# nitishsaDire/objectDetection_ssd

Hardware: NVIDIA B200
Metric: images/sec, SSD300 match + multibox loss fwd+bwd (higher is better)
Workload: dtype f32

## Files before the change

objectdetection_ssd_b200/csrc/common.cuh:

```cuda
#pragma once
#include <cuda_runtime.h>
#include <stdint.h>
#include <stdlib.h>
#include "../../include/ssdhead.h"

#if defined(__CUDA_ARCH__) && (__CUDA_ARCH__ < 1000)
#error "libssdhead is written for sm_100a (B200) only"
#endif

namespace ssdhead {

extern unsigned long long g_launch_count;
inline void count_launch(int n = 1) { g_launch_count += (unsigned long long)n; }

#define SSD_CHECK_CUDA(expr) do { cudaError_t _e = (expr); if (_e != cudaSuccess) return (int)_e; } while (0)
#define SSD_LAUNCH_CHECK() do { cudaError_t _e = cudaGetLastError(); if (_e != cudaSuccess) return (int)_e; } while (0)

static inline bool aligned16(const void* p) { return (reinterpret_cast<uintptr_t>(p) & 15u) == 0; }
static inline size_t round_up(size_t x, size_t a) { return (x + a - 1) / a * a; }

constexpr unsigned FULL = 0xffffffffu;

__device__ __forceinline__ float box_area(const float4 b) {
    return __fmul_rn(__fsub_rn(b.z, b.x), __fsub_rn(b.w, b.y));
// ... 8 lines not shown
    const float uni = __fsub_rn(__fadd_rn(area_a, area_b), inter);
    return __fdiv_rn(inter, uni);
}

__device__ __forceinline__ float iou_sparse(const float4 a, const float area_a, const float4 b, const float area_b) {
    const float lx = fmaxf(a.x, b.x), ly = fmaxf(a.y, b.y);
    const float hx = fminf(a.z, b.z), hy = fminf(a.w, b.w);
    const float dx = fmaxf(__fsub_rn(hx, lx), 0.0f);
    const float dy = fmaxf(__fsub_rn(hy, ly), 0.0f);
    const float inter = __fmul_rn(dx, dy);
    if (inter == 0.0f && area_a >= 0.0f) return 0.0f;
    return __fdiv_rn(inter, __fsub_rn(__fadd_rn(area_a, area_b), inter));
}

__device__ __forceinline__ float4 cxcywh_to_xyxy(const float4 b) {
    const float hw = __fdiv_rn(b.z, 2.0f), hh = __fdiv_rn(b.w, 2.0f);
    return make_float4(__fsub_rn(b.x, hw), __fsub_rn(b.y, hh), __fadd_rn(b.x, hw), __fadd_rn(b.y, hh));
}
__device__ __forceinline__ float4 xyxy_to_cxcywh(const float4 b) {
    return make_float4(__fdiv_rn(__fadd_rn(b.z, b.x), 2.0f), __fdiv_rn(__fadd_rn(b.w, b.y), 2.0f),
                       __fsub_rn(b.z, b.x), __fsub_rn(b.w, b.y));
}
__device__ __forceinline__ float4 encode_box(const float4 c, const float4 p) {
    return make_float4(__fdiv_rn(__fsub_rn(c.x, p.x), __fdiv_rn(p.z, 10.0f)),
                       __fdiv_rn(__fsub_rn(c.y, p.y), __fdiv_rn(p.w, 10.0f)),
                       __fmul_rn(logf(__fdiv_rn(c.z, p.z)), 5.0f),
                       __fmul_rn(logf(__fdiv_rn(c.w, p.w)), 5.0f));
}
__device__ __forceinline__ float4 decode_box(const float4 g, const float4 p) {
    return make_float4(__fadd_rn(__fdiv_rn(__fmul_rn(g.x, p.z), 10.0f), p.x),
                       __fadd_rn(__fdiv_rn(__fmul_rn(g.y, p.w), 10.0f), p.y),
                       __fmul_rn(expf(__fdiv_rn(g.z, 5.0f)), p.z),
                       __fmul_rn(expf(__fdiv_rn(g.w, 5.0f)), p.w));
}

__device__ __forceinline__ float fast_exp_ftz(float d) {
    float r;
    asm("ex2.approx.ftz.f32 %0, %1;" : "=f"(r) : "f"(__fmul_rn(d, 1.4426950408889634f)));
    return r;
}

__device__ __forceinline__ uint32_t float_order_key(float f) {
    f = __fadd_rn(f, 0.0f);
    const uint32_t u = __float_as_uint(f);
    return (u & 0x80000000u) ? ~u : (u | 0x80000000u);
}

__device__ __forceinline__ uint32_t smem_u32(const void* p) { return (uint32_t)__cvta_generic_to_shared(p); }

__device__ __forceinline__ void mbar_init(uint64_t* bar, uint32_t count) {
    asm volatile("mbarrier.init.shared::cta.b64 [%0], %1;" :: "r"(smem_u32(bar)), "r"(count) : "memory");
}
__device__ __forceinline__ void mbar_fence_init() {
    asm volatile("fence.mbarrier_init.release.cluster;" ::: "memory");
}
__device__ __forceinline__ void mbar_expect_tx(uint64_t* bar, uint32_t bytes) {
    asm volatile("mbarrier.arrive.expect_tx.shared::cta.b64 _, [%0], %1;" :: "r"(smem_u32(bar)), "r"(bytes) : "memory");
}
__device__ __forceinline__ void mbar_arrive(uint64_t* bar) {
    asm volatile("mbarrier.arrive.shared::cta.b64 _, [%0];" :: "r"(smem_u32(bar)) : "memory");
}
__device__ __forceinline__ void mbar_wait(uint64_t* bar, uint32_t parity) {
    asm volatile(
        "{\n\t.reg .pred p;\n\t"
        "WAIT_%=:\n\t"
        "mbarrier.try_wait.parity.shared::cta.b64 p, [%0], %1;\n\t"
        "@p bra DONE_%=;\n\t"
        "bra WAIT_%=;\n\t"
        "DONE_%=:\n\t}"
        :: "r"(smem_u32(bar)), "r"(parity) : "memory");
}
__device__ __forceinline__ void bulk_g2s(void* smem_dst, const void* gmem_src, uint32_t bytes, uint64_t* bar) {
    asm volatile("cp.async.bulk.shared::cluster.global.mbarrier::complete_tx::bytes [%0], [%1], %2, [%3];"
                 :: "r"(smem_u32(smem_dst)), "l"(gmem_src), "r"(bytes), "r"(smem_u32(bar)) : "memory");
}
__device__ __forceinline__ void bulk_s2g(void* gmem_dst, const void* smem_src, uint32_t bytes) {
    asm volatile("cp.async.bulk.global.shared::cta.bulk_group [%0], [%1], %2;"
                 :: "l"(gmem_dst), "r"(smem_u32(smem_src)), "r"(bytes) : "memory");
}
__device__ __forceinline__ void bulk_commit() { asm volatile("cp.async.bulk.commit_group;" ::: "memory"); }
__device__ __forceinline__ void bulk_wait_read_all() { asm volatile("cp.async.bulk.wait_group.read 0;" ::: "memory"); }
__device__ __forceinline__ void bulk_wait_all() { asm volatile("cp.async.bulk.wait_group 0;" ::: "memory"); }
__device__ __forceinline__ void fence_proxy_async_smem() { asm volatile("fence.proxy.async.shared::cta;" ::: "memory"); }

__device__ __forceinline__ uint64_t ld_cg_u64(const unsigned long long* p) {
    unsigned long long v;
    asm volatile("ld.global.cg.u64 %0, [%1];" : "=l"(v) : "l"(p) : "memory");
    return v;
}
__device__ __forceinline__ uint64_t ld_relaxed_gpu_u64(const unsigned long long* p) {
    unsigned long long v;
    asm volatile("ld.relaxed.gpu.global.u64 %0, [%1];" : "=l"(v) : "l"(p) : "memory");
    return v;
}
__device__ __forceinline__ int ld_relaxed_gpu_s32(const int* p) {
    int v;
    asm volatile("ld.relaxed.gpu.global.s32 %0, [%1];" : "=r"(v) : "l"(p) : "memory");
    return v;
}
__device__ __forceinline__ unsigned int ld_acquire_gpu_u32(const unsigned int* p) {
    unsigned int v;
    asm volatile("ld.acquire.gpu.global.u32 %0, [%1];" : "=r"(v) : "l"(p) : "memory");
    return v;
}
__device__ __forceinline__ void st_relaxed_gpu_u64(unsigned long long* p, unsigned long long v) {
    asm volatile("st.relaxed.gpu.global.u64 [%0], %1;" :: "l"(p), "l"(v) : "memory");
}
__device__ __forceinline__ unsigned short ld_cg_u16(const unsigned short* p) {
    unsigned short v;
    asm volatile("ld.global.cg.u16 %0, [%1];" : "=h"(v) : "l"(p) : "memory");
    return v;
}
__device__ __forceinline__ uint4 ld_cg_v4(const uint4* p) {
    uint4 v;
    asm volatile("ld.global.cg.v4.u32 {%0, %1, %2, %3}, [%4];" : "=r"(v.x), "=r"(v.y), "=r"(v.z), "=r"(v.w) : "l"(p) : "memory");
    return v;
}
__device__ __forceinline__ int ld_cg_s32(const int* p) {
    int v;
    asm volatile("ld.global.cg.s32 %0, [%1];" : "=r"(v) : "l"(p) : "memory");
    return v;
}

__device__ __forceinline__ void pdl_wait() { asm volatile("griddepcontrol.wait;" ::: "memory"); }
__device__ __forceinline__ void pdl_trigger() { asm volatile("griddepcontrol.launch_dependents;" ::: "memory"); }

template <bool COOP = false, typename... KArgs, typename... Args>
static inline cudaError_t launch_pdl(void (*kernel)(KArgs...), dim3 grid, dim3 block, size_t smem, cudaStream_t st, Args... args)
{
    cudaLaunchConfig_t cfg = {};
    cfg.gridDim = grid;
    cfg.blockDim = block;
    cfg.dynamicSmemBytes = smem;
    cfg.stream = st;
    cudaLaunchAttribute attr[2];
    attr[0].id = cudaLaunchAttributeProgrammaticStreamSerialization;
    attr[0].val.programmaticStreamSerializationAllowed = 1;
    attr[1].id = cudaLaunchAttributeCooperative;
    attr[1].val.cooperative = 1;
    cfg.attrs = attr;
    cfg.numAttrs = COOP ? 2 : 1;
    return cudaLaunchKernelEx(&cfg, kernel, KArgs(args)...);
}

struct MatchWs {
    unsigned long long* best_key;
    unsigned int* tile_counter;
    int* npos_acc;
    unsigned int* image_counter;
    unsigned long long* arrive_total;
};
static inline MatchWs match_ws(void* ws, int B, int sumG)
{
    uintptr_t w = (uintptr_t)ws;
    MatchWs m;
    m.best_key = (unsigned long long*)w;          w += round_up((size_t)sumG * 8, 16);
    m.tile_counter = (unsigned int*)w;            w += round_up((size_t)B * 4, 16);
    m.npos_acc = (int*)w;                         w += round_up((size_t)B * 4, 16);
    m.image_counter = (unsigned int*)w;
    m.arrive_total = (unsigned long long*)(w + 8);
    return m;
}
static inline size_t match_ws_bytes(int B, int sumG) { return (uintptr_t)match_ws(nullptr, B, sumG).image_counter + 16; }

__device__ __forceinline__ void st_release_sys_u64(unsigned long long* p, unsigned long long v) {
    asm volatile("st.release.sys.global.u64 [%0], %1;" :: "l"(p), "l"(v) : "memory");
// ... 32 lines not shown
```

objectdetection_ssd_b200/csrc/loss.cu:

```cuda
#include <algorithm>
#include <tuple>
#include <type_traits>
#include "common.cuh"

namespace ssdhead {

#ifdef SSDHEAD_PHASE_TIMES
__device__ long long g_phase_loss[16];
#define LPHASE(i) do { if (blockIdx.x == 0 && threadIdx.x == 0) g_phase_loss[i] = clock64(); } while (0)
__device__ long long g_cta[1024][12];
__device__ unsigned long long g_gt[8];
__device__ __forceinline__ unsigned long long gtimer() { unsigned long long v; asm volatile("mov.u64 %0, %globaltimer;" : "=l"(v)); return v; }
#define GMARK_MAX(i) do { if (threadIdx.x == 0) atomicMax(&g_gt[i], gtimer()); } while (0)
#define GMARK_MIN(i) do { if (threadIdx.x == 0) atomicMin(&g_gt[i], gtimer()); } while (0)
#else
#define LPHASE(i) do { } while (0)
#define GMARK_MAX(i) do { } while (0)
#define GMARK_MIN(i) do { } while (0)
#endif

template <int C, bool FAST = false>
__device__ __forceinline__ float row_cross_entropy(const float* __restrict__ row, int c)
{
    float x[C];
#pragma unroll
    for (int q = 0; q < C; ++q) x[q] = row[q];
    float m = x[0];
#pragma unroll
    for (int q = 1; q < C; ++q) m = fmaxf(m, x[q]);
    float s = 0.0f, xc = 0.0f;
#pragma unroll
    for (int q = 0; q < C; ++q) {
        const float d = __fsub_rn(x[q], m);
        s = __fadd_rn(s, FAST ? fast_exp_ftz(d) : expf(d));
        if (q == c) xc = d;
    }
    const float ce = __fsub_rn(logf(s), xc);
    return __fadd_rn(ce, 0.0f);
}

struct FusedMatch {
    const float4* gt_xyxy;
    const float* gt_cls;
    const int* gt_off;
    const float4* pri_xyxy;
    int P, bg_class;
    float pos_iou;
    uint8_t* cls_u8;
    unsigned long long* best_key;
    int* npos_acc;
    unsigned short* obj_u16;
    const float* seed_lb;
    int sumG;
};

struct FusedPre {
    float4 pb;
    float4 gbox;
    float gcls;
    int b, p;
    int b_first, b_last, off0, G;
};

__device__ __forceinline__ FusedPre fused_prefetch_bp(const FusedMatch& m, int b, int p, bool valid)
{
    FusedPre r;
    const int lane = threadIdx.x & 31;
    r.b = valid ? b : -1;
    r.p = valid ? p : 0;
    r.b_first = (int)__reduce_min_sync(FULL, valid ? (unsigned)r.b : 0x7fffffffu);
    r.b_last = __reduce_max_sync(FULL, r.b);
    r.pb = m.pri_xyxy[r.p];
    r.off0 = 0; r.G = 0;
    r.gbox = make_float4(0.f, 0.f, 0.f, 0.f);
    r.gcls = 0.0f;
    if (r.b_last >= 0) {
        r.off0 = m.gt_off[r.b_first];
        r.G = m.gt_off[r.b_first + 1] - r.off0;
        if (lane < min(r.G, 32)) { r.gbox = m.gt_xyxy[r.off0 + lane]; r.gcls = m.gt_cls[r.off0 + lane]; }
    }
    return r;
}

__device__ __forceinline__ FusedPre fused_prefetch(const FusedMatch& m, unsigned row, bool valid)
{
    const int b = (int)(row / (unsigned)m.P);
    return fused_prefetch_bp(m, b, (int)(row - (unsigned)b * (unsigned)m.P), valid);
}

template <bool MULTI = false>
__device__ __forceinline__ void fused_match_rows(const FusedMatch& m, unsigned row, bool valid, const FusedPre& pre)
{
    const int lane = threadIdx.x & 31;
    if (pre.b_last < 0) return;
    const int b = pre.b, p = pre.p;
    const float4 pb = pre.pb;
    const float pa = box_area(pb);
    if (MULTI && pre.b_last - pre.b_first >= 2) {
        if (valid) {
            const int off0 = m.gt_off[b], G = m.gt_off[b + 1] - off0;
            float bst = 0.0f;
            int obj_b = 0;
            float cls_b = G > 0 ? m.gt_cls[off0] : (float)m.bg_class;
            for (int g = 0; g < G; ++g) {
                const float4 gb = m.gt_xyxy[off0 + g];
                const float dx = __fsub_rn(fminf(gb.z, pb.z), fmaxf(gb.x, pb.x));
                const float dy = __fsub_rn(fminf(gb.w, pb.w), fmaxf(gb.y, pb.y));
                float v = 0.0f;
                if (dx > 0.0f && dy > 0.0f) {
                    const float inter = __fmul_rn(dx, dy);
                    v = __fdiv_rn(inter, __fsub_rn(__fadd_rn(box_area(gb), pa), inter));
                    if (v > bst) { bst = v; cls_b = m.gt_cls[off0 + g]; obj_b = g; }
                }
                if (v != 0.0f || p == 0)
                    atomicMax(&m.best_key[off0 + g],
                              ((unsigned long long)(__float_as_uint(v) | 0x80000000u) << 32) | (unsigned long long)(0xffffffffu - (uint32_t)p));
            }
            const bool hit = (G > 0) && !(bst < m.pos_iou);
            const int c = hit ? (int)cls_b : m.bg_class;
            m.cls_u8[row] = (uint8_t)c;
            if (m.obj_u16) m.obj_u16[row] = (unsigned short)obj_b;
            if (c != m.bg_class) atomicAdd(&m.npos_acc[b], 1);
        }
        return;
    }
    float best = 0.0f;
    int g_mine = 0, obj_mine = 0;
    float cls_mine = (float)m.bg_class;
    float wx1 = pb.x, wy1 = pb.y, wx2 = pb.z, wy2 = pb.w;
#pragma unroll
    for (int d = 16; d > 0; d >>= 1) {
        wx1 = fminf(wx1, __shfl_xor_sync(FULL, wx1, d));
        wy1 = fminf(wy1, __shfl_xor_sync(FULL, wy1, d));
        wx2 = fmaxf(wx2, __shfl_xor_sync(FULL, wx2, d));
        wy2 = fmaxf(wy2, __shfl_xor_sync(FULL, wy2, d));
    }
// ... 193 lines not shown
    int start[MAX_LEVELS + 1];
    int tile0[MAX_LEVELS + 1];
    int rows[MAX_LEVELS];
    int perm_stride, perm_inc;
    const float* conf[MAX_LEVELS];
    const float* loc[MAX_LEVELS];
    float* gconf[MAX_LEVELS];
    float* gloc[MAX_LEVELS];
};
__device__ __forceinline__ int level_of_tile(const LevelTab& lv, int vt) {
    int l = 0;
#pragma unroll
    for (int q = 1; q < MAX_LEVELS; ++q) if (q < lv.n && vt >= lv.tile0[q]) l = q;
    return l;
}
__device__ __forceinline__ int level_of_prior(const LevelTab& lv, int j) {
    int l = 0;
#pragma unroll
    for (int q = 1; q < MAX_LEVELS; ++q) if (q < lv.n && j >= lv.start[q]) l = q;
    return l;
}

template <int C, bool ZERO_FILL, bool MATCH, bool LEVELS>
__device__ __forceinline__ void
ce_stream_body(const float* __restrict__ conf, float* __restrict__ ce_out,
               float* __restrict__ grad_conf, float* __restrict__ grad_loc, long long total_rows, int use_tma,
               const FusedMatch& fm, const LevelTab* __restrict__ lvp)
{
    constexpr uint32_t TILE_BYTES = CE_ROWS * C * 4;
    constexpr uint32_t ZERO_BYTES = CE_ZERO_ROWS * C * 4;
    extern __shared__ __align__(128) unsigned char smem_raw[];
    __shared__ __align__(8) uint64_t s_full[CE_STAGES];
    __shared__ __align__(8) uint64_t s_empty[CE_STAGES];
    float* zero_tile = reinterpret_cast<float*>(smem_raw + (size_t)CE_STAGES * TILE_BYTES);

    const int t = threadIdx.x, lane = t & 31, warp = t >> 5;
    const long long full_tiles = LEVELS ? lvp->tile0[lvp->n] : (use_tma ? total_rows / CE_ROWS : 0);
    const int P = fm.P;

    if (t == 0) {
#pragma unroll
        for (int s = 0; s < CE_STAGES; ++s) { mbar_init(&s_full[s], 1); mbar_init(&s_empty[s], CE_ROWS / 32); }
        mbar_fence_init();
    }
    if (ZERO_FILL) {
        for (int i = t; i < (int)(ZERO_BYTES / 16); i += CE_THREADS)
            reinterpret_cast<float4*>(zero_tile)[i] = make_float4(0.f, 0.f, 0.f, 0.f);
        fence_proxy_async_smem();
    }
    pdl_trigger();
    pdl_wait();
    __syncthreads();

    if (warp == CE_ROWS / 32) {
        if (lane == 0) {
            int s = 0;
            uint32_t ph = 0;
            int vt = LEVELS ? (int)(((long long)blockIdx.x * lvp->perm_stride) % full_tiles) : 0;
            for (long long k = blockIdx.x; k < full_tiles; k += gridDim.x) {
                const long long tile = LEVELS ? (long long)vt : k;
                if (LEVELS) { vt += lvp->perm_inc; if (vt >= (int)full_tiles) vt -= (int)full_tiles; }
                mbar_wait(&s_empty[s], ph ^ 1u);
                const float* src = conf + (size_t)tile * CE_ROWS * C;
                float* gc = grad_conf + (size_t)tile * CE_ROWS * C;
                float* gl = grad_loc + (size_t)tile * CE_ROWS * 4;
                uint32_t nr = CE_ROWS;
                if (LEVELS) {
                    const int l = level_of_tile(*lvp, (int)tile);
                    const size_t r0 = (size_t)((int)tile - lvp->tile0[l]) * CE_ROWS;
                    nr = (uint32_t)min((long long)CE_ROWS, (long long)lvp->rows[l] - (long long)r0);
                    src = lvp->conf[l] + r0 * C;
                    if (ZERO_FILL) { gc = lvp->gconf[l] + r0 * C; gl = lvp->gloc[l] + r0 * 4; }
                }
                mbar_expect_tx(&s_full[s], nr * C * 4);
                bulk_g2s(smem_raw + (size_t)s * TILE_BYTES, src, nr * C * 4, &s_full[s]);
                if (ZERO_FILL) {
                    for (uint32_t o = 0; o < nr * C * 4; o += ZERO_BYTES)
                        bulk_s2g(reinterpret_cast<unsigned char*>(gc) + o, zero_tile, min(ZERO_BYTES, nr * C * 4 - o));
                    bulk_s2g(gl, zero_tile, nr * 16);
                    bulk_commit();
                }
                if (++s == CE_STAGES) { s = 0; ph ^= 1u; }
            }
            if (ZERO_FILL) bulk_wait_read_all();
        }
    } else {
        int s = 0;
        uint32_t ph = 0;
        FusedPre pre, nxt;
        if (!LEVELS) {
            if (MATCH && (long long)blockIdx.x < full_tiles) pre = fused_prefetch(fm, (unsigned)(blockIdx.x * CE_ROWS + t), true);
            for (long long tile = blockIdx.x; tile < full_tiles; tile += gridDim.x) {
                const long long row = tile * CE_ROWS + t;
                if (MATCH) {
                    if (tile + gridDim.x < full_tiles) nxt = fused_prefetch(fm, (unsigned)((tile + gridDim.x) * CE_ROWS + t), true);
                    fused_match_rows(fm, (unsigned)row, true, pre);
                    pre = nxt;
                }
                mbar_wait(&s_full[s], ph);
                const float ce = row_cross_entropy<C, true>(reinterpret_cast<const float*>(smem_raw + (size_t)s * TILE_BYTES) + t * C, C - 1);
                __syncwarp();
                if (lane == 0) mbar_arrive(&s_empty[s]);
                ce_out[row] = ce;
                if (++s == CE_STAGES) { s = 0; ph ^= 1u; }
            }
        } else {
            auto locate = [&](int tile, int& b, int& p) {
                const int l = level_of_tile(*lvp, tile);
                const unsigned lr = (unsigned)(tile - lvp->tile0[l]) * CE_ROWS + (unsigned)t, n = (unsigned)lvp->cnt[l];
                if (lr >= (unsigned)lvp->rows[l]) { b = -1; p = 0; return; }
                const unsigned bb = lr / n;
                b = (int)bb;
                p = lvp->start[l] + (int)(lr - bb * n);
            };
            int cb = -1, cp = 0, nb = -1, np = 0;
            const int T = (int)full_tiles;
            int vt = T > 0 ? (int)(((long long)blockIdx.x * lvp->perm_stride) % T) : 0;
            if ((long long)blockIdx.x < full_tiles) { locate(vt, cb, cp); pre = fused_prefetch_bp(fm, cb, cp, cb >= 0); }
            for (long long k = blockIdx.x; k < full_tiles; k += gridDim.x) {
                const bool valid = cb >= 0;
                const long long row = (long long)cb * P + cp;
                vt += lvp->perm_inc;
                if (vt >= T) vt -= T;
                if (k + gridDim.x < full_tiles) { locate(vt, nb, np); nxt = fused_prefetch_bp(fm, nb, np, nb >= 0); }
                fused_match_rows<true>(fm, (unsigned)row, valid, pre);
                pre = nxt;
                mbar_wait(&s_full[s], ph);
                float ce = 0.0f;
                if (valid) ce = row_cross_entropy<C, true>(reinterpret_cast<const float*>(smem_raw + (size_t)s * TILE_BYTES) + t * C, C - 1);
                __syncwarp();
                if (lane == 0) mbar_arrive(&s_empty[s]);
                if (valid) ce_out[row] = ce;
                cb = nb; cp = np;
                if (++s == CE_STAGES) { s = 0; ph ^= 1u; }
            }
        }
        if (!LEVELS) {
            const long long rest0 = full_tiles * CE_ROWS;
            for (long long row0 = rest0 + (long long)blockIdx.x * CE_ROWS; row0 < total_rows; row0 += (long long)gridDim.x * CE_ROWS) {
                const long long row = row0 + t;
                const bool valid = row < total_rows;
                if (MATCH) fused_match_rows(fm, (unsigned)row, valid, fused_prefetch(fm, (unsigned)row, valid));
                if (valid) {
                    ce_out[row] = row_cross_entropy<C, true>(conf + (size_t)row * C, C - 1);
                    if (ZERO_FILL) {
#pragma unroll
                        for (int q = 0; q < C; ++q) grad_conf[(size_t)row * C + q] = 0.0f;
#pragma unroll
                        for (int q = 0; q < 4; ++q) grad_loc[(size_t)row * 4 + q] = 0.0f;
                    }
                }
            }
        } else {
            for (int l = 0; l < lvp->n; ++l) {
                const unsigned n = (unsigned)lvp->cnt[l];
                const long long rows_l = total_rows / P * n;
                const long long rest0 = (long long)(lvp->tile0[l + 1] - lvp->tile0[l]) * CE_ROWS;
                const unsigned first = (blockIdx.x + gridDim.x - ((unsigned)l * (gridDim.x / MAX_LEVELS + 1)) % gridDim.x) % gridDim.x;
                for (long long r0 = rest0 + (long long)first * CE_ROWS; r0 < rows_l; r0 += (long long)gridDim.x * CE_ROWS) {
                    const long long lr = r0 + t;
                    const bool valid = lr < rows_l;
                    const unsigned b = valid ? (unsigned)(lr / n) : 0u;
                    const long long row = valid ? (long long)b * P + lvp->start[l] + (int)(lr - (long long)b * n) : total_rows;
                    if (MATCH) fused_match_rows<true>(fm, (unsigned)row, valid, fused_prefetch(fm, (unsigned)row, valid));
                    if (valid) {
                        ce_out[row] = row_cross_entropy<C, true>(lvp->conf[l] + (size_t)lr * C, C - 1);
                        if (ZERO_FILL) {
#pragma unroll
                            for (int q = 0; q < C; ++q) lvp->gconf[l][(size_t)lr * C + q] = 0.0f;
#pragma unroll
                            for (int q = 0; q < 4; ++q) lvp->gloc[l][(size_t)lr * 4 + q] = 0.0f;
                        }
                    }
                }
            }
        }
    }
    __syncthreads();
    GMARK_MAX(0);
}

template <int C, bool ZERO_FILL, bool MATCH>
__global__ void __launch_bounds__(CE_THREADS, CE_CTAS)
ce_stream_kernel(const float* __restrict__ conf, float* __restrict__ ce_out,
                 float* __restrict__ grad_conf, float* __restrict__ grad_loc, long long total_rows, int use_tma,
                 const FusedMatch fm)
{
    ce_stream_body<C, ZERO_FILL, MATCH, false>(conf, ce_out, grad_conf, grad_loc, total_rows, use_tma, fm, nullptr);
}

template <int C, bool ZERO_FILL>
__global__ void __launch_bounds__(CE_THREADS, CE_CTAS)
ce_stream_levels_kernel(float* __restrict__ ce_out, long long total_rows, const FusedMatch fm, const __grid_constant__ LevelTab lv)
{
    ce_stream_body<C, ZERO_FILL, true, true>(nullptr, ce_out, nullptr, nullptr, total_rows, 1, fm, &lv);
}

constexpr int MN_T = 512;
constexpr int MN_W = MN_T / 32;
constexpr int MN_BINS = 2048;

struct MineParams {
    const float* loc;
    const float* conf;
    const float* ce;
    float* ce_w;
    float* ce_tap;
    const uint8_t* cls_u8;
    const float4* gt_xyxy;
    const float* gt_cls;
    const int* gt_off;
    const float4* pri_xyxy;
    const float4* pri_cxcywh;
    const int* best_prior;
    const int* npos;
    const int* npos_norm;
    int B, P, neg_ratio, bg_class;
    float pos_iou;
    double* sums;
    float* losses;
    float* grad_loc;
    float* grad_conf;
    uint32_t* mined_mask;
    double* partials;
    unsigned int* done_counter;
    unsigned short* obj_u16;
    uint8_t* cls_rw;
    int* best_prior_w;
    int* npos_w;
    unsigned long long* best_key;
    int* npos_acc;
    unsigned long long* arrive_total;
    int xchg_R, xchg_rank;
    unsigned int xchg_seq;
    unsigned long long* const* xchg_peers;
    unsigned long long* xchg_local;
    int* err_flag;
    float* sp_conf;
    float* sp_loc;
    int* sp_idx;
    int* sp_cnt;
    int sp_cap;
    unsigned char* res_base;
    size_t res_stride;
};


__device__ __forceinline__ uint32_t block_exclusive_scan(uint32_t v, uint32_t* s_warp , uint32_t* total)
{
    const int lane = threadIdx.x & 31, warp = threadIdx.x >> 5;
    uint32_t inc = v;
#pragma unroll
    for (int d = 1; d < 32; d <<= 1) {
        const uint32_t o = __shfl_up_sync(FULL, inc, d);
        if (lane >= d) inc += o;
    }
    __syncthreads();
    if (lane == 31) s_warp[warp] = inc;
    __syncthreads();
    uint32_t base = 0u, tot = 0u;
#pragma unroll
    for (int w = 0; w < MN_W; ++w) { const uint32_t c = s_warp[w]; if (w < warp) base += c; tot += c; }
    *total = tot;
    return base + inc - v;
}

constexpr int MN_GC = 64;
constexpr int MN_CAND = 512;

template <int C, bool GRADS, bool FIN, bool LEVELS, bool SPARSE = false>
__device__ __forceinline__ void mine_body(const MineParams& p, const LevelTab* __restrict__ lvp)
{
    extern __shared__ __align__(128) unsigned char smem_raw[];
    uint32_t* s_key = reinterpret_cast<uint32_t*>(smem_raw);
    uint32_t* s_hist = s_key + p.P;
    uint16_t* s_list = reinterpret_cast<uint16_t*>(s_hist + MN_BINS);
    uint8_t* s_cls = reinterpret_cast<uint8_t*>(s_list + ((p.P + 7) & ~7));
    __shared__ uint32_t s_warp[MN_W + 1];
    __shared__ uint32_t s_sel[3];
    __shared__ uint32_t s_nsel, s_ncand, s_max;
    __shared__ uint32_t s_npl;
    __shared__ uint32_t s_ckey[MN_CAND], s_cidx[MN_CAND];
    __shared__ float4 s_gbox[MN_GC];
    __shared__ float s_garea[MN_GC];
    __shared__ int s_gbp[MN_GC];
    __shared__ double s_redd[2][MN_W];

    const int b = blockIdx.x, t = threadIdx.x, lane = t & 31, warp = t >> 5;
    const int P = p.P;
    const size_t row0 = (size_t)b * P;
    const int off0 = p.gt_off[b];
    const int G = p.gt_off[b + 1] - off0;
    double acc_l1 = 0.0, acc_ce = 0.0;
    auto conf_row = [&](int j) -> const float* {
        if (!LEVELS) return p.conf + (row0 + j) * C;
        const int l = level_of_prior(*lvp, j);
        return lvp->conf[l] + ((size_t)b * lvp->cnt[l] + (size_t)(j - lvp->start[l])) * C;
    };
    auto gconf_row = [&](int j) -> float* {
        if (!LEVELS) return p.grad_conf + (row0 + j) * C;
        const int l = level_of_prior(*lvp, j);
        return lvp->gconf[l] + ((size_t)b * lvp->cnt[l] + (size_t)(j - lvp->start[l])) * C;
    };
    auto loc_row = [&](int j) -> const float4* {
        if (!LEVELS) return reinterpret_cast<const float4*>(p.loc) + row0 + j;
        const int l = level_of_prior(*lvp, j);
        return reinterpret_cast<const float4*>(lvp->loc[l]) + (size_t)b * lvp->cnt[l] + (size_t)(j - lvp->start[l]);
    };
    auto gloc_row = [&](int j) -> float4* {
        if (!LEVELS) return reinterpret_cast<float4*>(p.grad_loc) + row0 + j;
        const int l = level_of_prior(*lvp, j);
        return reinterpret_cast<float4*>(lvp->gloc[l]) + (size_t)b * lvp->cnt[l] + (size_t)(j - lvp->start[l]);
    };

    if (t == 0) { s_nsel = 0u; s_ncand = 0u; s_max = 0u; s_npl = 0u; }
    if (t < min(G, MN_GC)) {
        const float4 bx = p.gt_xyxy[off0 + t];
        s_gbox[t] = bx;
        s_garea[t] = box_area(bx);
    }
    pdl_trigger();
    pdl_wait();
    __syncthreads();
    int* res_cnt = nullptr;
    unsigned short* res_rows = nullptr;
    if (GRADS && !SPARSE && p.res_base) {
        res_cnt = reinterpret_cast<int*>(p.res_base + (size_t)b * p.res_stride);
        res_rows = reinterpret_cast<unsigned short*>(p.res_base + (size_t)b * p.res_stride + 8);
        const int n_prev = res_cnt[0], npl_prev = res_cnt[1];
        for (int i = t; i < n_prev; i += MN_T) {
            const int j = (int)res_rows[i];
            float* g = gconf_row(j);
#pragma unroll
            for (int q = 0; q < C; ++q) g[q] = 0.0f;
            if (i < npl_prev) *gloc_row(j) = make_float4(0.f, 0.f, 0.f, 0.f);
        }
    }
    LPHASE(0);
    GMARK_MIN(1); GMARK_MAX(2);
#ifdef SSDHEAD_PHASE_TIMES
    const long long cta_t0 = clock64();
#endif
    int acc0 = 0;
    unsigned long long bk0 = 0ull;
    if (FIN) {
        acc0 = ld_cg_s32(&p.npos_acc[b]);
        if (t < G) bk0 = ld_cg_u64(&p.best_key[off0 + t]);
    }
    uint32_t kmax = 0u;
    const bool vec_ok = ((P & 3) == 0) && (((row0 * 4) & 15) == 0) && ((reinterpret_cast<uintptr_t>(p.ce) & 15) == 0) &&
                        ((reinterpret_cast<uintptr_t>(p.cls_u8) & 3) == 0);
    if (vec_ok) {
        const float4* ce4 = reinterpret_cast<const float4*>(p.ce + row0);
        const uchar4* cl4 = reinterpret_cast<const uchar4*>(p.cls_u8 + row0);
        const int nvec = P >> 2;
        constexpr int KU = 5;
        for (int v0 = t; v0 < nvec; v0 += KU * MN_T) {
            float4 e5[KU];
            uchar4 c5[KU];
#pragma unroll
            for (int u = 0; u < KU; ++u) {
                const int v = v0 + u * MN_T;
                if (v < nvec) { e5[u] = ce4[v]; c5[u] = cl4[v]; }
            }
#pragma unroll
            for (int u = 0; u < KU; ++u) {
                const int v = v0 + u * MN_T;
                if (v >= nvec) break;
                const float4 e = e5[u];
                const uchar4 c = c5[u];
                const float ev[4] = {e.x, e.y, e.z, e.w};
                const uint8_t cv[4] = {c.x, c.y, c.z, c.w};
                uint32_t kv[4];
#pragma unroll
                for (int q = 0; q < 4; ++q) {
                    const bool pos = (int)cv[q] != p.bg_class;
                    kv[q] = pos ? 0u : (__float_as_uint(ev[q]) & 0x7fffffffu);
                    kmax = max(kmax, kv[q]);
                }
                reinterpret_cast<uint4*>(s_key)[v] = make_uint4(kv[0], kv[1], kv[2], kv[3]);
                reinterpret_cast<uchar4*>(s_cls)[v] = c;
            }
        }
    } else {
        for (int j = t; j < P; j += MN_T) {
            const float ce = p.ce[row0 + j];
            const uint8_t c = p.cls_u8[row0 + j];
            const bool pos = (int)c != p.bg_class;
            const uint32_t key = pos ? 0u : (__float_as_uint(ce) & 0x7fffffffu);
            s_key[j] = key;
            s_cls[j] = c;
            kmax = max(kmax, key);
        }
    }
    kmax = __reduce_max_sync(FULL, kmax);
    if (lane == 0) atomicMax(&s_max, kmax);
    LPHASE(1);
    int npos_b;
    if (FIN) {
        __shared__ int s_fin_extra, s_fin_npos;
        if (t == 0) s_fin_extra = 0;
        for (int g = t; g < G; g += MN_T) {
            const unsigned long long bkv = g == t ? bk0 : ld_cg_u64(&p.best_key[off0 + g]);
            const int bp = (int)(0xffffffffu - (uint32_t)(bkv & 0xffffffffull));
            p.best_key[off0 + g] = 0ull;
// ... 339 lines not shown
#pragma unroll
            for (int i = 0; i < C; ++i) {
                const int e = lane + 32 * i, r = e / C, q = e - r * C;
                float* rp;
                if (SPARSE) {
                    rp = p.sp_conf + ((size_t)b * p.sp_cap + (wbase + (uint32_t)r)) * C;
                    if (r < nrw && wbase + (uint32_t)r < (uint32_t)p.sp_cap) rp[q] = v[i];
                    continue;
                }
                if (LEVELS) rp = reinterpret_cast<float*>(__shfl_sync(FULL, (unsigned long long)my_grow, r));
                else rp = gconf_row(__shfl_sync(FULL, j, r));
                if (r < nrw) rp[q] = v[i];
            }
            __syncwarp();
        }
#ifdef SSDHEAD_PHASE_TIMES
        if (lane == 0 && warp == 0 && b < 1024 && base < 2 * MN_T) g_cta[b][9 + base / MN_T] = clock64() - cta_t0;
#endif
#ifdef SSDHEAD_PHASE_TIMES
        __syncwarp();
        if (lane == 0 && (warp == 0 || warp == MN_W - 1) && b < 1024 && base < 2 * MN_T)
            g_cta[b][5 + (warp ? 2 : 0) + base / MN_T] = clock64() - cta_t0;
#endif
    }

#ifdef SSDHEAD_PHASE_TIMES
    if (t == 0 && b < 1024) g_cta[b][1] = clock64() - cta_t0;
#endif
    LPHASE(5);
    acc_l1 = warp_sum(acc_l1);
    acc_ce = warp_sum(acc_ce);
    if (lane == 0) { s_redd[0][warp] = acc_l1; s_redd[1][warp] = acc_ce; }
    __syncthreads();
    __shared__ int s_is_last;
    if (t == MN_T - 1) {
        double a = 0.0, c = 0.0;
        for (int w = 0; w < MN_W; ++w) { a += s_redd[0][w]; c += s_redd[1][w]; }
        p.partials[2 * b] = a;
        p.partials[2 * b + 1] = c;
        __threadfence();
        const unsigned done = atomicAdd(p.done_counter, 1u);
        s_is_last = (done == gridDim.x - 1u) ? 1 : 0;
    }
    __syncthreads();
    LPHASE(6);
    if (s_is_last) {
        __threadfence();
        double a = 0.0, c = 0.0;
        for (int s = t; s < (int)gridDim.x; s += MN_T) {
            a += __longlong_as_double((long long)ld_relaxed_gpu_u64(reinterpret_cast<const unsigned long long*>(p.partials) + 2 * (size_t)s));
            c += __longlong_as_double((long long)ld_relaxed_gpu_u64(reinterpret_cast<const unsigned long long*>(p.partials) + 2 * (size_t)s + 1));
        }
        a = warp_sum(a);
        c = warp_sum(c);
        __syncthreads();
        if (lane == 0) { s_redd[0][warp] = a; s_redd[1][warp] = c; }
        __syncthreads();
        if (t == 0) {
            a = 0.0; c = 0.0;
            for (int w = 0; w < MN_W; ++w) { a += s_redd[0][w]; c += s_redd[1][w]; }
            if (FIN && p.xchg_R > 1) {
                for (int q = 0; q < p.xchg_R; ++q) {
                    st_relaxed_sys_u64(p.xchg_peers[q] + xchg_slot(p.xchg_seq, 1, p.xchg_rank), (unsigned long long)__double_as_longlong(a));
                    st_relaxed_sys_u64(p.xchg_peers[q] + xchg_slot(p.xchg_seq, 2, p.xchg_rank), (unsigned long long)__double_as_longlong(c));
                }
                __threadfence_system();
                for (int q = 0; q < p.xchg_R; ++q)
                    st_relaxed_sys_u64(p.xchg_peers[q] + xchg_slot(p.xchg_seq, 3, p.xchg_rank), (unsigned long long)p.xchg_seq);
                unsigned spins = 0;
                a = 0.0; c = 0.0;
                for (int q = 0; q < p.xchg_R; ++q) {
                    while ((unsigned)ld_acquire_sys_u64(p.xchg_local + xchg_slot(p.xchg_seq, 3, q)) != p.xchg_seq && ++spins < (1u << 27)) __nanosleep(64);
                    a += __longlong_as_double((long long)ld_relaxed_sys_u64(p.xchg_local + xchg_slot(p.xchg_seq, 1, q)));
                    c += __longlong_as_double((long long)ld_relaxed_sys_u64(p.xchg_local + xchg_slot(p.xchg_seq, 2, q)));
                }
                if (spins >= (1u << 27)) *p.err_flag = 1;
            }
            p.sums[0] = a;
            p.sums[1] = c;
            const double N = (double)npos_total;
            p.losses[0] = (float)(a / (4.0 * N));
            p.losses[1] = (float)(c / N);
            *p.done_counter = 0u;
            if (FIN) {
                p.npos_w[p.B] = (p.xchg_R > 1) ? (int)(unsigned)ld_cg_u64(p.arrive_total) : npos_total;
                *p.arrive_total = 0ull;
            }
        }
    }
    GMARK_MAX(3);
#ifdef SSDHEAD_PHASE_TIMES
    if (t == 0 && b < 1024) g_cta[b][2] = clock64() - cta_t0;
#endif
}


template <int C, bool GRADS, bool FIN>
__global__ void __launch_bounds__(MN_T, 2)
mine_kernel(const MineParams p)
{
    mine_body<C, GRADS, FIN, false>(p, nullptr);
}

template <int C>
__global__ void __launch_bounds__(MN_T, 2)
mine_sparse_kernel(const MineParams p)
{
    mine_body<C, true, false, false, true>(p, nullptr);
}

template <int C, bool GRADS, bool FIN>
__global__ void __launch_bounds__(MN_T, 2)
mine_levels_kernel(const MineParams p, const __grid_constant__ LevelTab lv)
{
    mine_body<C, GRADS, FIN, true>(p, &lv);
}


__global__ void finish_loss_kernel(const double* __restrict__ sums, const int* __restrict__ npos_norm, float* __restrict__ losses)
{
    const double N = (double)(*npos_norm);
    losses[0] = (float)(sums[0] / (4.0 * N));
    losses[1] = (float)(sums[1] / N);
}

__global__ void __launch_bounds__(256)
scale_grads_kernel(float4* __restrict__ gl, size_t n4_loc, float* __restrict__ gl_tail, int tail_loc,
                   float4* __restrict__ gc, size_t n4_conf, float* __restrict__ gc_tail, int tail_conf,
                   const float* __restrict__ gout)
{
    const float a = gout[0], c = gout[1];
    if (a == 1.0f && c == 1.0f) return;
    const size_t stride = (size_t)gridDim.x * blockDim.x;
    const size_t tid = (size_t)blockIdx.x * blockDim.x + threadIdx.x;
    if (a != 1.0f) {
        for (size_t i = tid; i < n4_loc; i += stride) { float4 v = gl[i]; v.x *= a; v.y *= a; v.z *= a; v.w *= a; gl[i] = v; }
        if (tid < (size_t)tail_loc) gl_tail[tid] *= a;
    }
    if (c != 1.0f) {
        for (size_t i = tid; i < n4_conf; i += stride) { float4 v = gc[i]; v.x *= c; v.y *= c; v.z *= c; v.w *= c; gc[i] = v; }
        if (tid < (size_t)tail_conf) gc_tail[tid] *= c;
    }
}

static size_t mine_smem_bytes(int P) { return (size_t)P * 4 + MN_BINS * 4 + (size_t)((P + 7) & ~7) * 2 + round_up((size_t)P, 16); }

struct LossWs {
    unsigned int* done_counter;
    double* partials;
    float* ce;
    unsigned short* obj;
    float* seed;
};
static LossWs loss_ws(void* ws, int B, int P)
{
    uintptr_t w = (uintptr_t)ws;
    LossWs l;
    l.done_counter = (unsigned int*)w;            w += 16;
    l.partials = (double*)w;                      w += round_up((size_t)B * 2 * sizeof(double), 16);
    l.ce = (float*)w;                             w += round_up((size_t)B * P * sizeof(float), 16);
    l.obj = (unsigned short*)w;                   w += round_up((size_t)B * P * sizeof(unsigned short), 16);
    l.seed = (float*)w;
    return l;
}
size_t loss_workspace_bytes(int B, int P, int C)
{
    if (mine_smem_bytes(P) > 220 * 1024 || P >= 65536) return 0;
    return (uintptr_t)loss_ws(nullptr, B, P).seed + (size_t)SEED_CAP * sizeof(float);
}
size_t loss_ws_header_bytes(int maxB) { return (uintptr_t)loss_ws(nullptr, maxB, 0).ce + 256; }

static size_t resident_row_stride(int P) { return round_up(8 + (size_t)P * sizeof(unsigned short), 16); }
size_t resident_rows_bytes(int B, int P)
{
    if (B <= 0 || P <= 0 || P >= 65536) return 0;
    return (size_t)B * resident_row_stride(P);
}

static int g_num_sms = 0;
static int num_sms()
{
    if (g_num_sms == 0) {
        int dev = 0, n = 0;
        if (cudaGetDevice(&dev) != cudaSuccess || cudaDeviceGetAttribute(&n, cudaDevAttrMultiProcessorCount, dev) != cudaSuccess || n <= 0) n = 148;
        g_num_sms = n;
    }
    return g_num_sms;
}

template <int C, bool GRADS, bool MATCH>
static int launch_ce_stream(const float* conf, float* ce, float* grad_conf, float* grad_loc, long long rows,
                            const FusedMatch& fm, const LevelTab* lv, cudaStream_t st)
{
    constexpr size_t tile = (size_t)CE_ROWS * C * 4;
    const size_t smem_ce = tile * CE_STAGES + (GRADS ? (size_t)CE_ZERO_ROWS * C * 4 : 0);
    const long long tiles = (rows + CE_ROWS - 1) / CE_ROWS + (lv ? lv->n : 0);
    const int grid_ce = (int)std::min<long long>(tiles, (long long)CE_CTAS * num_sms());
    if (MATCH && fm.seed_lb) {
        const int stride = std::max(SEED_STRIDE, (fm.P + SEED_MAX - 1) / SEED_MAX);
        const int nsamp = (fm.P + stride - 1) / stride;
        const size_t smem_seed = (size_t)nsamp * 16;
        SSD_CHECK_CUDA(cudaFuncSetAttribute(match_seed_kernel, cudaFuncAttributeMaxDynamicSharedMemorySize, (int)smem_seed));
        const int grid_seed = std::min((fm.sumG + 7) / 8, 2 * num_sms());
        const int B = (int)(rows / fm.P);
        match_seed_kernel<<<grid_seed, 256, smem_seed, st>>>(fm.gt_xyxy, fm.gt_off, B, fm.pri_xyxy, nsamp, stride,
                                                             const_cast<float*>(fm.seed_lb));
        SSD_LAUNCH_CHECK();
        count_launch();
    }
    if (MATCH && lv) {
        auto kce = ce_stream_levels_kernel<C, GRADS>;
        SSD_CHECK_CUDA(cudaFuncSetAttribute(kce, cudaFuncAttributeMaxDynamicSharedMemorySize, (int)smem_ce));
        LevelTab lt = *lv;
        const long long T = lt.tile0[lt.n];
        auto gcd = [](long long a, long long b) { while (b) { const long long c = a % b; a = b; b = c; } return a; };
        long long S = std::max<long long>(1, (long long)(0.6180339887 * (double)T));
        while (S > 1 && gcd(S, T) != 1) --S;
        lt.perm_stride = (int)S;
        lt.perm_inc = T > 0 ? (int)(((long long)grid_ce * S) % T) : 0;
        SSD_CHECK_CUDA(launch_pdl(kce, dim3(grid_ce), dim3(CE_THREADS), smem_ce, st, ce, rows, fm, lt));
    } else {
        auto kce = ce_stream_kernel<C, GRADS, MATCH>;
        SSD_CHECK_CUDA(cudaFuncSetAttribute(kce, cudaFuncAttributeMaxDynamicSharedMemorySize, (int)smem_ce));
        const int use_tma = (aligned16(conf) && (!GRADS || (aligned16(grad_conf) && aligned16(grad_loc)))) ? 1 : 0;
        SSD_CHECK_CUDA(launch_pdl(kce, dim3(grid_ce), dim3(CE_THREADS), smem_ce, st, conf, ce, grad_conf, grad_loc, rows, use_tma, fm));
    }
    count_launch();
    return 0;
}

static bool stream_capturing(cudaStream_t st)
{
    cudaStreamCaptureStatus cs = cudaStreamCaptureStatusNone;
    if (cudaStreamIsCapturing(st, &cs) != cudaSuccess) {
        (void)cudaGetLastError();
        return true;
    }
    return cs != cudaStreamCaptureStatusNone;
}

template <typename... KArgs>
static int mine_fits_coresident(void (*kmn)(KArgs...), int B, int P, bool* fits)
{
    const size_t smem_mn = mine_smem_bytes(P);
    SSD_CHECK_CUDA(cudaFuncSetAttribute(kmn, cudaFuncAttributeMaxDynamicSharedMemorySize, (int)smem_mn));
    int per_sm = 0;
    SSD_CHECK_CUDA(cudaOccupancyMaxActiveBlocksPerMultiprocessor(&per_sm, kmn, MN_T, smem_mn));
    *fits = (long long)per_sm * num_sms() >= B;
    return 0;
}

template <bool FIN, typename... KArgs, typename... Args>
static int launch_mine(void (*kmn)(KArgs...), int B, int P, cudaStream_t st, Args... args)
{
    const size_t smem_mn = mine_smem_bytes(P);
    if (!FIN) {
        SSD_CHECK_CUDA(cudaFuncSetAttribute(kmn, cudaFuncAttributeMaxDynamicSharedMemorySize, (int)smem_mn));
        SSD_CHECK_CUDA(launch_pdl(kmn, dim3(B), dim3(MN_T), smem_mn, st, args...));
        count_launch();
        return 0;
    }
    bool fits = false;
    const int rc = mine_fits_coresident(kmn, B, P, &fits);
    if (rc || !fits) return rc ? rc : 1;
    static int with_pdl = 0;
    const bool capturing = with_pdl >= 0 && stream_capturing(st);
    if (with_pdl == 1 || (with_pdl == 0 && !capturing)) {
        const cudaError_t e = launch_pdl<true>(kmn, dim3(B), dim3(MN_T), smem_mn, st, args...);
        if (e == cudaSuccess) { with_pdl = 1; count_launch(); return 0; }
        if (capturing) return (int)e;
        (void)cudaGetLastError();
        with_pdl = -1;
    }
    static_assert(std::is_same<std::tuple<std::decay_t<Args>...>, std::tuple<std::decay_t<KArgs>...>>::value,
                  "the cooperative launch passes the arguments by address: they must have the kernel's parameter types");
    void* ptrs[] = {(void*)&args...};
    SSD_CHECK_CUDA(cudaLaunchCooperativeKernel((const void*)kmn, dim3(B), dim3(MN_T), ptrs, smem_mn, st));
    count_launch();
    return 0;
}
// ... 74 lines not shown
    lv->n = levels->num_levels;
    int sum = 0, with_grads = 0;
    int t0 = 0;
    for (int l = 0; l < lv->n; ++l) {
        const int n = levels->count[l];
        if (n <= 0 || !levels->conf[l] || !levels->loc[l]) return SSDHEAD_E_BADARG;
        if (!aligned16(levels->loc[l])) return SSDHEAD_E_ALIGN;
        const bool g = levels->grad_conf[l] != nullptr;
        if (g != (levels->grad_loc[l] != nullptr)) return SSDHEAD_E_BADARG;
        if (g && !aligned16(levels->grad_loc[l])) return SSDHEAD_E_ALIGN;
        const bool tma_ok = aligned16(levels->conf[l]) && (!g || aligned16(levels->grad_conf[l]));
        with_grads += g ? 1 : 0;
        lv->cnt[l] = n; lv->start[l] = sum; lv->tile0[l] = t0;
        lv->conf[l] = levels->conf[l]; lv->loc[l] = levels->loc[l]; lv->gconf[l] = levels->grad_conf[l]; lv->gloc[l] = levels->grad_loc[l];
        sum += n;
        const long long rows_l = (long long)B * n;
        lv->rows[l] = (int)rows_l;
        if (tma_ok) t0 += (int)(rows_l / CE_ROWS) + ((rows_l % CE_ROWS) != 0 && (rows_l % 4) == 0 ? 1 : 0);
    }
    for (int l = lv->n; l <= MAX_LEVELS; ++l) { lv->start[l] = sum; lv->tile0[l] = t0; }
    if (sum != P) return SSDHEAD_E_BADARG;
    if (with_grads != 0 && with_grads != lv->n) return SSDHEAD_E_BADARG;
    return 0;
}

static FusedMatch bind_match(const StepArgs& a, const MatchWs& mw, unsigned short* obj_u16, const float* seed_lb)
{
    FusedMatch fm = {};
    fm.gt_xyxy = (const float4*)a.gt_xyxy; fm.gt_cls = a.gt_cls; fm.gt_off = a.gt_off; fm.pri_xyxy = (const float4*)a.pri_xyxy;
    fm.P = a.P; fm.bg_class = a.C - 1; fm.pos_iou = a.pos_iou; fm.cls_u8 = a.cls_u8; fm.best_key = mw.best_key; fm.npos_acc = mw.npos_acc;
    fm.obj_u16 = obj_u16; fm.sumG = a.sumG; fm.seed_lb = seed_lb;
    return fm;
}

static MineParams bind_mine(const StepArgs& a, const LossWs& lw, const int32_t* npos_norm, const MatchWs* mw)
{
    MineParams prm = {};
    prm.loc = a.loc; prm.conf = a.conf; prm.cls_u8 = a.cls_u8;
    prm.gt_xyxy = (const float4*)a.gt_xyxy; prm.gt_cls = a.gt_cls; prm.gt_off = a.gt_off;
    prm.pri_xyxy = (const float4*)a.pri_xyxy; prm.pri_cxcywh = (const float4*)a.pri_cxcywh;
    prm.best_prior = a.best_prior; prm.npos = a.npos; prm.npos_norm = npos_norm;
    prm.B = a.B; prm.P = a.P; prm.neg_ratio = a.neg_ratio; prm.bg_class = a.C - 1; prm.pos_iou = a.pos_iou;
    prm.sums = a.sums; prm.losses = a.losses; prm.grad_loc = a.grad_loc; prm.grad_conf = a.grad_conf;
    prm.mined_mask = a.mined_mask;
    prm.done_counter = lw.done_counter;
    prm.partials = lw.partials;
    prm.ce = a.ce ? a.ce : lw.ce;
    prm.ce_tap = a.ce;
    if (mw) {
        prm.cls_rw = a.cls_u8; prm.best_prior_w = a.best_prior; prm.npos_w = a.npos;
        prm.best_key = mw->best_key; prm.npos_acc = mw->npos_acc; prm.arrive_total = mw->arrive_total;
    }
    return prm;
}

static int launch_finalize(const StepArgs& a, const MatchWs& mw, cudaStream_t st)
{
    match_finalize_kernel<<<a.B, 64, 0, st>>>(a.gt_cls, a.gt_off, a.B, a.P, a.C - 1, a.best_prior, a.npos, a.cls_u8,
                                              mw.best_key, mw.npos_acc, mw.image_counter);
    SSD_LAUNCH_CHECK();
    count_launch();
    return 0;
}

template <bool GRADS>
static int launch_mine_step(const StepArgs& a, const MineParams& prm, const LevelTab* lv, const MatchWs& mw, cudaStream_t st)
{
    int rc = lv ? launch_mine<true>(mine_levels_kernel<21, GRADS, true>, a.B, a.P, st, prm, *lv)
                : launch_mine<true>(mine_kernel<21, GRADS, true>, a.B, a.P, st, prm);
    if (rc != 1) return rc;
    if (prm.xchg_R > 1) return SSDHEAD_E_UNSUPPORTED;
    rc = launch_finalize(a, mw, st);
    if (rc) return rc;
    return lv ? launch_mine<false>(mine_levels_kernel<21, GRADS, false>, a.B, a.P, st, prm, *lv)
              : launch_mine<false>(mine_kernel<21, GRADS, false>, a.B, a.P, st, prm);
}

static int step_impl(const StepArgs& a, const LevelTab* lv, const Xchg& x, void* ws_rows)
{
    cudaStream_t st = (cudaStream_t)a.stream;
    const LossWs lw = loss_ws(a.ws_loss, a.B, a.P);
    const MatchWs mw = match_ws(a.ws_match, a.B, a.sumG);
    unsigned short* obj = a.sumG <= 65535 ? lw.obj : nullptr;
    const FusedMatch fm = bind_match(a, mw, obj, !lv && match_cull_enabled(a.B, a.sumG) ? lw.seed : nullptr);
    MineParams prm = bind_mine(a, lw, a.npos + a.B, &mw);
    prm.obj_u16 = obj;
    prm.xchg_R = x.R; prm.xchg_rank = x.rank; prm.xchg_seq = x.seq;
    prm.xchg_peers = (unsigned long long* const*)x.peers; prm.xchg_local = (unsigned long long*)x.local; prm.err_flag = x.err_flag;
    if (ws_rows) {
        prm.res_base = (unsigned char*)ws_rows;
        prm.res_stride = resident_row_stride(a.P);
    }
    if (lv) prm.ce_w = lw.ce;
    const bool grads = lv ? lv->gconf[0] != nullptr : a.grad_loc != nullptr;
    if (x.R > 1) {
        bool fits = false;
        const int frc = lv ? (grads ? mine_fits_coresident(mine_levels_kernel<21, true, true>, a.B, a.P, &fits)
                                    : mine_fits_coresident(mine_levels_kernel<21, false, true>, a.B, a.P, &fits))
                           : (grads ? mine_fits_coresident(mine_kernel<21, true, true>, a.B, a.P, &fits)
                                    : mine_fits_coresident(mine_kernel<21, false, true>, a.B, a.P, &fits));
        if (frc) return frc;
        if (!fits) return SSDHEAD_E_UNSUPPORTED;
    }
    const bool ce_grads = grads && !ws_rows;
    const long long rows = (long long)a.B * a.P;
    float* ce = a.ce ? a.ce : lw.ce;
    int rc = ce_grads ? launch_ce_stream<21, true, true>(a.conf, ce, a.grad_conf, a.grad_loc, rows, fm, lv, st)
                      : launch_ce_stream<21, false, true>(a.conf, ce, nullptr, nullptr, rows, fm, lv, st);
    if (rc) return rc;
    if (a.mined_mask) SSD_CHECK_CUDA(cudaMemsetAsync(a.mined_mask, 0, (size_t)a.B * ((a.P + 31) / 32) * sizeof(uint32_t), st));
    return grads ? launch_mine_step<true>(a, prm, lv, mw, st) : launch_mine_step<false>(a, prm, lv, mw, st);
}

static int step_flat(const StepArgs& a, const Xchg& x, void* ws_rows)
{
    int rc = check_mine(a, true);
    if (!rc && (!aligned16(a.loc) || !aligned16(a.pri_cxcywh))) rc = SSDHEAD_E_ALIGN;
    if (!rc) rc = check_match(a);
    if (rc || a.B == 0) return rc;
    return step_impl(a, nullptr, x, ws_rows);
}

static int step_levels(const ssdhead_levels* levels, const StepArgs& a, const Xchg& x)
{
    LevelTab lv = {};
    int rc = check_mine(a, false);
    if (!rc) rc = check_match(a);
    if (!rc) rc = check_levels(levels, a.B, a.P, &lv);
    if (rc || a.B == 0) return rc;
    if (!aligned16(a.pri_cxcywh)) return SSDHEAD_E_ALIGN;
    return step_impl(a, &lv, x, nullptr);
}

}

using namespace ssdhead;

extern "C" {

int ssdhead_ce_stream(const float* conf, int B, int P, int C, float* ce, float* grad_loc, float* grad_conf,
                      void* ws, size_t ws_bytes, void* stream)
{
    if (!conf) return SSDHEAD_E_BADARG;
    const int rc = check_loss(B, P, C, grad_loc, grad_conf, ws, ws_bytes);
    if (rc || B == 0) return rc;
    float* ce_buf = ce ? ce : loss_ws(ws, B, P).ce;
    const long long rows = (long long)B * P;
    FusedMatch none = {};
    return grad_loc ? launch_ce_stream<21, true, false>(conf, ce_buf, grad_conf, grad_loc, rows, none, nullptr, (cudaStream_t)stream)
                    : launch_ce_stream<21, false, false>(conf, ce_buf, nullptr, nullptr, rows, none, nullptr, (cudaStream_t)stream);
}

int ssdhead_ce_match_stream(const float* conf, const float* gt_xyxy, const float* gt_cls, const int32_t* gt_off,
                            const float* pri_xyxy, int B, int P, int C, int sumG, float pos_iou,
                            float* ce, float* grad_loc, float* grad_conf,
                            uint8_t* cls_u8, int32_t* best_prior, int32_t* npos,
                            void* ws_loss, size_t ws_loss_bytes, void* ws_match, size_t ws_match_bytes,
                            int run_finalizer, void* stream)
{
    const StepArgs a = {.conf = conf, .gt_xyxy = gt_xyxy, .gt_cls = gt_cls, .gt_off = gt_off, .pri_xyxy = pri_xyxy,
                        .B = B, .P = P, .C = C, .sumG = sumG, .pos_iou = pos_iou, .grad_loc = grad_loc,
                        .grad_conf = grad_conf, .cls_u8 = cls_u8, .best_prior = best_prior, .npos = npos, .ce = ce,
                        .ws_loss = ws_loss, .ws_loss_bytes = ws_loss_bytes, .ws_match = ws_match,
                        .ws_match_bytes = ws_match_bytes, .stream = stream};
    if (!conf) return SSDHEAD_E_BADARG;
    int rc = check_match(a);
    if (rc || B == 0) return rc;
    cudaStream_t st = (cudaStream_t)stream;
    const LossWs lw = loss_ws(ws_loss, B, P);
    const MatchWs mw = match_ws(ws_match, B, sumG);
    const FusedMatch fm = bind_match(a, mw, nullptr, match_cull_enabled(B, sumG) ? lw.seed : nullptr);
    float* ce_buf = ce ? ce : lw.ce;
    const long long rows = (long long)B * P;
    rc = grad_loc ? launch_ce_stream<21, true, true>(conf, ce_buf, grad_conf, grad_loc, rows, fm, nullptr, st)
                  : launch_ce_stream<21, false, true>(conf, ce_buf, nullptr, nullptr, rows, fm, nullptr, st);
    if (rc || !run_finalizer) return rc;
    return launch_finalize(a, mw, st);
}

int ssdhead_multibox_step(const float* loc, const float* conf,
                          const float* gt_xyxy, const float* gt_cls, const int32_t* gt_off,
                          const float* pri_xyxy, const float* pri_cxcywh,
                          int B, int P, int C, int sumG, int neg_ratio, float pos_iou,
                          double* sums, float* losses, float* grad_loc, float* grad_conf,
                          uint8_t* cls_u8, int32_t* best_prior, int32_t* npos,
// ... 205 lines not shown
```

Measured before the change: 2.448 million.

## Replace PDL grid wait with per-CTA completion counter between CE stream and mine

```diff
diff --git a/objectdetection_ssd_b200/csrc/common.cuh b/objectdetection_ssd_b200/csrc/common.cuh
--- a/objectdetection_ssd_b200/csrc/common.cuh
+++ b/objectdetection_ssd_b200/csrc/common.cuh
@@ -114,6 +114,7 @@
 __device__ __forceinline__ void bulk_wait_read_all() { asm volatile("cp.async.bulk.wait_group.read 0;" ::: "memory"); }
 __device__ __forceinline__ void bulk_wait_all() { asm volatile("cp.async.bulk.wait_group 0;" ::: "memory"); }
 __device__ __forceinline__ void fence_proxy_async_smem() { asm volatile("fence.proxy.async.shared::cta;" ::: "memory"); }
+__device__ __forceinline__ void fence_proxy_async_global() { asm volatile("fence.proxy.async.global;" ::: "memory"); }
 
 __device__ __forceinline__ uint64_t ld_cg_u64(const unsigned long long* p) {
     unsigned long long v;
diff --git a/objectdetection_ssd_b200/csrc/loss.cu b/objectdetection_ssd_b200/csrc/loss.cu
--- a/objectdetection_ssd_b200/csrc/loss.cu
+++ b/objectdetection_ssd_b200/csrc/loss.cu
@@ -52,6 +52,7 @@
     unsigned short* obj_u16;
     const float* seed_lb;
     int sumG;
+    unsigned int* ctas_done;
 };
 
 struct FusedPre {
@@ -411,7 +412,15 @@
                 }
                 if (++s == CE_STAGES) { s = 0; ph ^= 1u; }
             }
-            if (ZERO_FILL) bulk_wait_read_all();
+            if (ZERO_FILL) {
+                if (fm.ctas_done) {
+                    bulk_wait_all();
+                    fence_proxy_async_global();
+                    __threadfence();
+                } else {
+                    bulk_wait_read_all();
+                }
+            }
         }
     } else {
         int s = 0;
@@ -506,6 +515,10 @@
         }
     }
     __syncthreads();
+    if (!LEVELS && fm.ctas_done && t == 0) {
+        __threadfence();
+        atomicAdd(fm.ctas_done, 1u);
+    }
     GMARK_MAX(0);
 }
 
@@ -560,6 +573,8 @@
     unsigned long long* best_key;
     int* npos_acc;
     unsigned long long* arrive_total;
+    unsigned int* stream_done;
+    unsigned int stream_ctas;
     int xchg_R, xchg_rank;
     unsigned int xchg_seq;
     unsigned long long* const* xchg_peers;
@@ -649,7 +664,16 @@
         s_garea[t] = box_area(bx);
     }
     pdl_trigger();
-    pdl_wait();
+    if (FIN && p.stream_done) {
+        if (t == 0) {
+            unsigned spins = 0;
+            while (ld_acquire_gpu_u32(p.stream_done) < p.stream_ctas && ++spins < (1u << 22)) __nanosleep(32);
+            if (spins >= (1u << 22)) pdl_wait();
+            __threadfence();
+        }
+    } else {
+        pdl_wait();
+    }
     __syncthreads();
     int* res_cnt = nullptr;
     unsigned short* res_rows = nullptr;
@@ -1155,12 +1179,14 @@
             p.losses[0] = (float)(a / (4.0 * N));
             p.losses[1] = (float)(c / N);
             *p.done_counter = 0u;
+            if (FIN && p.stream_done) *p.stream_done = 0u;
             if (FIN) {
                 p.npos_w[p.B] = (p.xchg_R > 1) ? (int)(unsigned)ld_cg_u64(p.arrive_total) : npos_total;
                 *p.arrive_total = 0ull;
             }
         }
     }
+    if (FIN && p.stream_done) pdl_wait();
     GMARK_MAX(3);
 #ifdef SSDHEAD_PHASE_TIMES
     if (t == 0 && b < 1024) g_cta[b][2] = clock64() - cta_t0;
@@ -1220,6 +1246,7 @@
 
 struct LossWs {
     unsigned int* done_counter;
+    unsigned int* ctas_done;
     double* partials;
     float* ce;
     unsigned short* obj;
@@ -1229,7 +1256,8 @@
 {
     uintptr_t w = (uintptr_t)ws;
     LossWs l;
-    l.done_counter = (unsigned int*)w;            w += 16;
+    l.done_counter = (unsigned int*)w;
+    l.ctas_done = (unsigned int*)(w + 4);         w += 16;
     l.partials = (double*)w;                      w += round_up((size_t)B * 2 * sizeof(double), 16);
     l.ce = (float*)w;                             w += round_up((size_t)B * P * sizeof(float), 16);
     l.obj = (unsigned short*)w;                   w += round_up((size_t)B * P * sizeof(unsigned short), 16);
@@ -1261,14 +1289,19 @@
     return g_num_sms;
 }
 
+static int ce_stream_grid(long long rows, const LevelTab* lv)
+{
+    const long long tiles = (rows + CE_ROWS - 1) / CE_ROWS + (lv ? lv->n : 0);
+    return (int)std::min<long long>(tiles, (long long)CE_CTAS * num_sms());
+}
+
 template <int C, bool GRADS, bool MATCH>
 static int launch_ce_stream(const float* conf, float* ce, float* grad_conf, float* grad_loc, long long rows,
                             const FusedMatch& fm, const LevelTab* lv, cudaStream_t st)
 {
     constexpr size_t tile = (size_t)CE_ROWS * C * 4;
     const size_t smem_ce = tile * CE_STAGES + (GRADS ? (size_t)CE_ZERO_ROWS * C * 4 : 0);
-    const long long tiles = (rows + CE_ROWS - 1) / CE_ROWS + (lv ? lv->n : 0);
-    const int grid_ce = (int)std::min<long long>(tiles, (long long)CE_CTAS * num_sms());
+    const int grid_ce = ce_stream_grid(rows, lv);
     if (MATCH && fm.seed_lb) {
         const int stride = std::max(SEED_STRIDE, (fm.P + SEED_MAX - 1) / SEED_MAX);
         const int nsamp = (fm.P + stride - 1) / stride;
@@ -1509,7 +1542,7 @@
     const LossWs lw = loss_ws(a.ws_loss, a.B, a.P);
     const MatchWs mw = match_ws(a.ws_match, a.B, a.sumG);
     unsigned short* obj = a.sumG <= 65535 ? lw.obj : nullptr;
-    const FusedMatch fm = bind_match(a, mw, obj, !lv && match_cull_enabled(a.B, a.sumG) ? lw.seed : nullptr);
+    FusedMatch fm = bind_match(a, mw, obj, !lv && match_cull_enabled(a.B, a.sumG) ? lw.seed : nullptr);
     MineParams prm = bind_mine(a, lw, a.npos + a.B, &mw);
     prm.obj_u16 = obj;
     prm.xchg_R = x.R; prm.xchg_rank = x.rank; prm.xchg_seq = x.seq;
@@ -1528,6 +1561,16 @@
                                     : mine_fits_coresident(mine_kernel<21, false, true>, a.B, a.P, &fits));
         if (frc) return frc;
         if (!fits) return SSDHEAD_E_UNSUPPORTED;
+    } else if (!lv) {
+        bool fits = false;
+        const int frc = grads ? mine_fits_coresident(mine_kernel<21, true, true>, a.B, a.P, &fits)
+                              : mine_fits_coresident(mine_kernel<21, false, true>, a.B, a.P, &fits);
+        if (frc) return frc;
+        if (fits) {
+            fm.ctas_done = lw.ctas_done;
+            prm.stream_done = lw.ctas_done;
+            prm.stream_ctas = (unsigned)ce_stream_grid((long long)a.B * a.P, nullptr);
+        }
     }
     const bool ce_grads = grads && !ws_rows;
     const long long rows = (long long)a.B * a.P;
```

New measurement: 2.219 million (median of 6 runs). 9.4% lower.
